# duanzhiihao/lossy-vae

Measured on AMD Instinct MI355X. Metric: Mpixels/s enc+dec (qarv_base, 512x768), higher is better.
Workload: dtype f32 (2-term fp16 split of every fp32 operand, hi + lo*2^-11 = 23 of 24 significant bits; 3 fp16 MFMAs per product step in two fp32 accumulators: fp32-class accuracy, parity-tested); 1 GPU; qarv_base batch=8 512x768 synthetic per GPU, compress_batch+decompress_batch, HIP kernels (f16x2) + host rANS, seeded random-init weights (profile typical); global_batch=8, parallelism=dp1 (images sharded, no data-path collective)

## Files before the change

lossy-vae_amd/csrc/gemm_h2_choice.h:

```cpp
#pragma once

#include "../../include/lvae_hip.h"

namespace lvae_h2 {

struct Choice {
    int kernel;
    int params[5];
    int splitk;
};

inline int slices(const lvae_gemm_desc& d) { return d.ksplit > 1 ? d.ksplit : 1; }

inline bool h2n_takes(const lvae_gemm_desc& d, bool force, Choice* c) {
    const bool conv3 = d.a_mode == LVAE_A_CONV3;
    if (d.prec != 4 || d.a_h2 || d.a_gelu || d.out_h2 || (d.a_mode != LVAE_A_PLAIN && !conv3) || d.N > 96 || (d.K & 15) || d.ldw != d.K) return false;
    if (!conv3 && (d.K1 != 0 || d.K0 != d.K || (d.lda0 & 3) || (long)d.M * d.lda0 * 4 > 0x7ffffff0L)) return false;
    if (conv3 && ((d.K0 & 15) || d.K != 9 * d.K0 || d.K1 != 0 || d.H <= 0 || d.W <= 0 || (long)d.M * d.K0 * 4 > 0x7ffffff0L)) return false;
    if ((long)d.N * d.K * 4 > 0x7ffffff0L) return false;
    const int S = slices(d);
    if (S > 1 && ((d.K / 16) % S || d.store != LVAE_ST_ROWMAJOR || (d.N & 3) || (d.ldo & 3) || (d.ldres & 3))) return false;
    if (!force && !(d.K & 16) && !(d.M >= 32768 && S == 1 && (conv3 || d.N > 64))) return false;
    *c = Choice{2, {(d.N + 31) / 32, conv3 ? LVAE_A_CONV3 : LVAE_A_PLAIN, 0, 0, 0}, 0};
    return true;
// ... 17 lines not shown
    if (sel <= 0 || sel > 2) {
        double best = 1e300;
        const double eff[3] = {0, 0.70, 1.00};
        for (int tn = 1; tn <= 2; ++tn) {
            const long tiles = (long)((M + 127) / 128) * ((N + 64 * tn - 1) / (64 * tn)) * S;
            const long rounds = (tiles + 511) / 512;
            const double cost = rounds * (128.0 * 64 * tn) * (K + 96.0) / eff[tn];
            if (cost < best) { best = cost; sel = tn; }
        }
    }
    *c = Choice{1, {sel, d.a_gelu ? 1 : 0, d.a_mode, 0, 0}, 0};
    return true;
}

inline bool h2p_takes(const lvae_gemm_desc& d, int force, int cu_count, Choice* c) {
    if (d.prec != 4 || !d.a_h2 || d.a_mode != LVAE_A_PLAIN || d.K1 != 0 || d.K0 != d.K || (d.K & 31) || d.lda0 != d.K ||
        d.ldw != d.K || d.a_gelu || (long)256 * d.K * 4 > 0x7fffffffL)
        return false;
    const int M = d.M, N = d.N;
    if (d.ksplit > 1) {
        if ((d.K / 32) % d.ksplit || d.store != LVAE_ST_ROWMAJOR || (N & 3) || (d.ldo & 3) || (d.ldres & 3)) return false;
        const int tiles = ((M + 127) / 128) * ((N + 63) / 64);
        const bool loaders = tiles <= cu_count;
        *c = Choice{3, {2, 1, 3, 1, loaders ? 8 : 0}, 0};
        return true;
    }
    int sel = force;
    if (sel != 42 && sel != 41 && sel != 22 && sel != 21 && sel != 23) {
        const int tn = (N % 128 == 0 || ((N + 127) / 128) * 128 - N < ((N + 63) / 64) * 64 - N + 1) ? 2 : 1;
        const long t128 = (long)((M + 127) / 128) * ((N + 127) / 128);
        sel = tn == 1 ? 21 : (t128 < 1024 ? 21 : (t128 >= 4096 ? 42 : 22));
        const long t64 = (long)((M + 127) / 128) * ((N + 63) / 64);
        if (d.K <= 512 && t64 >= 512 && (sel == 21 || (sel == 22 && t128 < 2048))) sel = 23;
    }
    switch (sel) {
        case 42: *c = Choice{3, {4, 2, 3, 0, 0}, 0}; break;
        case 41: *c = Choice{3, {4, 1, 3, 0, 0}, 0}; break;
        case 22: *c = Choice{3, {2, 2, 2, 0, 0}, 0}; break;
        case 23: *c = Choice{3, {2, 1, 2, 0, 0}, 0}; break;
        default: *c = Choice{3, {2, 1, 3, 0, 0}, 0}; break;
    }
    return true;
}

inline int family(const lvae_gemm_desc& d, int cu_count, Choice* c) {
    if (d.out_h2 && (d.store != LVAE_ST_ROWMAJOR || (d.epi != LVAE_EPI_BIAS && d.epi != LVAE_EPI_BIAS_GELU) || (d.N & 31) ||
                     d.ldo != d.N || (d.ksplit > 1 && !d.a_h2)))
        return -22;
    const int force = d.cfg > 0 ? d.cfg : 0;
    if (d.a_h2) return h2p_takes(d, force, cu_count, c) ? 0 : -22;
    return h2_takes(d, force, c) ? 0 : -22;
}

inline int choose(const lvae_gemm_desc& d, int cu_count, Choice* out) {
    if (d.prec != 4 || d.M <= 0 || d.N <= 0 || d.K <= 0 || (d.K & 7) || (d.ldw & 7)) return -22;
    if ((d.epi == LVAE_EPI_GAMMA_RES || d.epi == LVAE_EPI_RES) && !d.res) return -22;
    if (d.epi == LVAE_EPI_GAMMA_RES && !d.gamma) return -22;
    if (d.store != LVAE_ST_ROWMAJOR && (d.r <= 0 || d.N % (d.r * d.r) || d.H <= 0 || d.W <= 0)) return -22;
    const int S = slices(d);
    Choice c{};
    int rc;
    if (S == 1) {
        rc = family(d, cu_count, &c);
    } else if (d.a_h2) {
        if (d.store != LVAE_ST_ROWMAJOR || (d.N & 3) || (d.ldo & 3) || (d.ldres & 3) || d.K % (32 * S)) return -22;
        rc = family(d, cu_count, &c);
        c.splitk = 1;
    } else if ((d.cfg == 0 || d.cfg == 3) && h2n_takes(d, d.cfg == 3, &c)) {
        rc = 0;
        c.splitk = 1;
    } else {
        if (!d.ws || d.store != LVAE_ST_ROWMAJOR || (d.N & 3) || (d.ldo & 3) || (d.ldres & 3) || d.K % (32 * S)) return -22;
        rc = family(d, cu_count, &c);
        c.splitk = (d.cnt && ((d.N & 31) == 0 || d.N <= 32)) ? 2 : d.defer_reduce ? 4 : 3;
    }
    if (rc) return rc;
    *out = c;
    return 0;
// ... 4 lines not shown
```

lossy-vae_amd/csrc/gemm_h2p.hip:

```cpp
#include "gemm_common.h"

#include <type_traits>

namespace {

typedef _Float16 f16x8 __attribute__((ext_vector_type(8)));

#define LVAE_FENCE() __builtin_amdgcn_sched_barrier(0)
#define H2P_DSR(dst, addr, off) asm volatile("ds_read_b128 %0, %1 offset:%2" : "=v"(dst) : "v"(addr), "n"(off))
#define H2P_MFMA(a, b, c) __builtin_amdgcn_mfma_f32_32x32x16_f16(a, b, c, 0, 0, 0)

template <int WM, int TN, int NBUF, bool FOLD = false, int NLOAD = 0>
__global__ __launch_bounds__(128 * WM + 64 * NLOAD, (NLOAD ? 1 : (WM == 4 ? 1 : (NBUF == 2 && TN == 1 ? 3 : 2)))) void gemm_h2p_kernel(const lvae_gemm_desc d, int tiles_n, int n_tiles, int stagger) {
    using C = Cfg<WM, 2, 2, TN, 1, 32>;
    constexpr int BM = 64 * WM, BN = 64 * TN, ROWS = BM + BN, STAGE = ROWS * 128;
    constexpr int NWAVE = 2 * WM, NG = ROWS / 8, NI = NG / NWAVE;
    static_assert(NG % NWAVE == 0 && NWAVE % 2 == 0, "whole DMA instructions per wave; g has the parity of the wave");
    static_assert(NBUF * STAGE <= 160 * 1024 / (NLOAD ? 1 : (WM == 4 ? 1 : (NBUF == 2 && TN == 1 ? 3 : 2))), "LDS");
    static_assert(NLOAD == 0 || (NLOAD % 2 == 0 && NG % NLOAD == 0 && (NBUF - 2) * (NG / (NLOAD ? NLOAD : 1)) <= 63), "whole pieces per loader wave; the piece index has the loader's parity");
    extern __shared__ __attribute__((aligned(16))) float smem[];
    int t;
    {
        const int b = blockIdx.x, q = n_tiles / 8, r = n_tiles % 8, xcd = b % 8, loc = b / 8;
        t = (xcd < r ? xcd * (q + 1) : r * (q + 1) + (xcd - r) * q) + loc;
    }
    const int tm = t / tiles_n, tn = t - tm * tiles_n;
    const int m0 = tm * BM, n0 = tn * BN;
    const int tid = threadIdx.x, lane = tid & 63;
    const int wave = __builtin_amdgcn_readfirstlane(tid >> 6);
    const int wave_m = wave >> 1, wave_n = wave & 1;
    const int li = lane & 31, lh = lane >> 5;
    const int nq = d.K / 32;
    const int rowb = d.K * 4;
    if (stagger > 0) {
        const bool late = WM == 4 ? ((__builtin_amdgcn_s_getreg(((4 - 1) << 11) | (8 << 6) | 4) & 1) != 0)
                                  : (__builtin_amdgcn_s_getreg(((8 - 1) << 11) | (0 << 6) | 6) != 0);
        if (late)
            for (int i = 0; i < nq * stagger; ++i) __builtin_amdgcn_s_sleep(8);
    }

    const int rows_a = (d.M - m0) < BM ? (d.M - m0) : BM, rows_w = (d.N - n0) < BN ? (d.N - n0) : BN;
    const __amdgpu_buffer_rsrc_t rsA =
        __builtin_amdgcn_make_buffer_rsrc((void*)((const char*)d.A0 + (long)m0 * rowb), 0, rows_a * rowb, 0x00020000);
    const __amdgpu_buffer_rsrc_t rsW =
        __builtin_amdgcn_make_buffer_rsrc((void*)((const char*)d.Wt16 + (long)n0 * rowb), 0, rows_w * rowb, 0x00020000);
    if constexpr (NLOAD > 0) {
        if (wave >= NWAVE) {
// ... 12 lines not shown
                }
            };
#pragma unroll
            for (int s = 0; s < NBUF - 1; ++s) issue(s < nq ? s : nq - 1, s);
            int nb = NBUF - 1;
            for (int s = 0; s < nq; ++s) {
                asm volatile("s_waitcnt vmcnt(%0)\n\ts_barrier" ::"n"((NBUF - 2) * PL) : "memory");
                issue(s + NBUF - 1 < nq ? s + NBUF - 1 : nq - 1, nb);
                nb = nb == NBUF - 1 ? 0 : nb + 1;
            }
            asm volatile("s_waitcnt vmcnt(0)\n\ts_barrier" ::: "memory");
            return;
        }
    }
    const int r_in = lane >> 3, pp = lane & 7;
    const int dvoff = r_in * rowb + ((pp ^ ((4 * (wave & 1) + (r_in >> 1)) & 7)) << 4);
    auto dma = [&](int i, int stage, int buf) {
        const int g = i * NWAVE + wave;
        const bool isA = g < BM / 8;
        const int soff = (isA ? 8 * g : 8 * g - BM) * rowb + stage * 128;
        __builtin_amdgcn_raw_ptr_buffer_load_lds(isA ? rsA : rsW, (__attribute__((address_space(3))) void*)((char*)smem + buf * STAGE + g * 1024),
                                                 16, dvoff, soff, 0, 0);
    };

    const int xr = (li >> 1) & 7;
    unsigned a_base[4], b_base[4];
#pragma unroll
    for (int pt = 0; pt < 4; ++pt) {
        const int piece = 4 * (pt >> 1) + 2 * (pt & 1) + lh;
        const unsigned o = (unsigned)((piece ^ xr) << 4);
        a_base[pt] = (unsigned)(unsigned long)(__attribute__((address_space(3))) char*)((char*)smem) + (wave_m * 64 + li) * 128 + o;
        b_base[pt] = (unsigned)(unsigned long)(__attribute__((address_space(3))) char*)((char*)smem) + (BM + wave_n * 32 * TN + li) * 128 + o;
    }

    f32x16 accH[2][TN], accX[2][TN];
#pragma unroll
    for (int a = 0; a < 2; ++a)
// ... 12 lines not shown
            for (int a = 0; a < 2; ++a)
#pragma unroll
                for (int b = 0; b < TN; ++b)
#pragma unroll
                    for (int r = 0; r < 16; ++r) {
                        const float pr = __builtin_fmaf(accX[a][b][r], 1.0f / 2048.0f, accH[a][b][r]) + 0.0f;
                        tot[a][b][r] = slice == 0 ? pr : tot[a][b][r] + pr;
                        accH[a][b][r] = 0.f; accX[a][b][r] = 0.f;
                    }
            ++slice;
        }
    };

    if constexpr (NLOAD == 0) {
#pragma unroll
        for (int s = 0; s < NBUF - 1; ++s)
#pragma unroll
            for (int i = 0; i < NI; ++i) dma(i, s < nq ? s : nq - 1, s);
    }

    f16x8 af[2][2][2], bf[2][TN][2];
    auto stage_body = [&](auto buf_tag, int s) {
        constexpr int BUF = decltype(buf_tag)::value, NXT = (BUF + NBUF - 1) % NBUF;
        if constexpr (NLOAD > 0) asm volatile("s_barrier" ::: "memory");
        else asm volatile("s_waitcnt vmcnt(%0)\n\ts_barrier" ::"n"((NBUF - 2) * NI) : "memory");
        LVAE_FENCE();
        unsigned aa[4], ba[4];
#pragma unroll
        for (int pt = 0; pt < 4; ++pt) { aa[pt] = a_base[pt] + BUF * STAGE; ba[pt] = b_base[pt] + BUF * STAGE; }
#pragma unroll
        for (int tt = 0; tt < 2; ++tt) {
#pragma unroll
            for (int a = 0; a < 2; ++a) {
                H2P_DSR(af[tt][a][0], aa[0 + tt], a * 4096);
                H2P_DSR(af[tt][a][1], aa[2 + tt], a * 4096);
            }
#pragma unroll
            for (int b = 0; b < TN; ++b) {
                H2P_DSR(bf[tt][b][0], ba[0 + tt], b * 4096);
                H2P_DSR(bf[tt][b][1], ba[2 + tt], b * 4096);
            }
        }
        const int sn = s + NBUF - 1 < nq ? s + NBUF - 1 : nq - 1;
        int issued = 0;
#pragma unroll
        for (int tt = 0; tt < 2; ++tt) {
            if (tt == 0) {
                if constexpr (TN == 2) asm volatile("s_waitcnt lgkmcnt(8)" : "+v"(af[0][0][0]), "+v"(af[0][0][1]), "+v"(af[0][1][0]), "+v"(af[0][1][1]),
                                                    "+v"(bf[0][0][0]), "+v"(bf[0][0][1]), "+v"(bf[0][1][0]), "+v"(bf[0][1][1]));
                else asm volatile("s_waitcnt lgkmcnt(6)" : "+v"(af[0][0][0]), "+v"(af[0][0][1]), "+v"(af[0][1][0]), "+v"(af[0][1][1]),
                                  "+v"(bf[0][0][0]), "+v"(bf[0][0][1]));
            } else {
                if constexpr (TN == 2) asm volatile("s_waitcnt lgkmcnt(0)" : "+v"(af[1][0][0]), "+v"(af[1][0][1]), "+v"(af[1][1][0]), "+v"(af[1][1][1]),
                                                    "+v"(bf[1][0][0]), "+v"(bf[1][0][1]), "+v"(bf[1][1][0]), "+v"(bf[1][1][1]));
                else asm volatile("s_waitcnt lgkmcnt(0)" : "+v"(af[1][0][0]), "+v"(af[1][0][1]), "+v"(af[1][1][0]), "+v"(af[1][1][1]),
                                  "+v"(bf[1][0][0]), "+v"(bf[1][0][1]));
            }
            LVAE_FENCE();
// ... 6 lines not shown
                        accX[1][b] = H2P_MFMA(af[tt][1][1], bf[tt][b][0], accX[1][b]);
                    } else if (j == 1) {
                        accX[0][b] = H2P_MFMA(af[tt][0][0], bf[tt][b][1], accX[0][b]);
                        accX[1][b] = H2P_MFMA(af[tt][1][0], bf[tt][b][1], accX[1][b]);
                    } else {
                        accH[0][b] = H2P_MFMA(af[tt][0][0], bf[tt][b][0], accH[0][b]);
                        accH[1][b] = H2P_MFMA(af[tt][1][0], bf[tt][b][0], accH[1][b]);
                    }
                    if constexpr (NLOAD == 0) { if (issued < NI) { dma(issued, sn, NXT); ++issued; } }
                    LVAE_FENCE();
                }
            }
        }
        static_assert(NI <= 6 * TN, "DMA instructions per stage must fit the MFMA pairs of a stage");
    };
    for (int s = 0; s < nq; s += NBUF) {
        stage_body(std::integral_constant<int, 0>{}, s);
        fold();
        if (s + 1 < nq) { stage_body(std::integral_constant<int, 1 % NBUF>{}, s + 1); fold(); }
        if (NBUF > 2 && s + 2 < nq) { stage_body(std::integral_constant<int, 2 % NBUF>{}, s + 2); fold(); }
    }
    asm volatile("s_waitcnt vmcnt(0)\n\ts_barrier" ::: "memory");
    if constexpr (FOLD) {
        if (d.bias && n0 + BN <= d.N && !((d.ldo | d.ldres) & 3)) {
            if (d.epi == LVAE_EPI_BIAS_GELU && d.out_h2 && !(d.ldo & 31)) {
                h2p_epilogue_fast<TN, LVAE_EPI_BIAS_GELU, true, true, true>(d, tot, m0, n0, rows_a, wave_m, wave_n, li, lh);
                return;
            }
            if (d.epi == LVAE_EPI_GAMMA_RES && !d.out_h2) {
                h2p_epilogue_fast<TN, LVAE_EPI_GAMMA_RES, false, false, true>(d, tot, m0, n0, rows_a, wave_m, wave_n, li, lh);
                return;
            }
            if (d.epi == LVAE_EPI_RES && !d.out_h2) {
                h2p_epilogue_fast<TN, LVAE_EPI_RES, false, false, true>(d, tot, m0, n0, rows_a, wave_m, wave_n, li, lh);
                return;
            }
        }
        const int lj = li & 3;
#pragma unroll
        for (int a = 0; a < 2; ++a)
#pragma unroll
            for (int g = 0; g < 4; ++g) {
                const int row = m0 + (wave_m * 2 + a) * 32 + 4 * lh + 8 * g + lj;
// ... 1 lines not shown
                for (int b = 0; b < TN; ++b) {
                    float v0 = tot[a][b][4 * g + 0], v1 = tot[a][b][4 * g + 1], v2 = tot[a][b][4 * g + 2], v3 = tot[a][b][4 * g + 3];
                    quad_transpose(v0, v1, v2, v3, lj);
                    const int c4 = n0 + (wave_n * TN + b) * 32 + (li & ~3);
                    if (row < d.M && c4 < d.N) splitk_epilogue_store<true>(d, row, c4, (f32x4){v0, v1, v2, v3});
                }
            }
        return;
    }
#pragma unroll
    for (int a = 0; a < 2; ++a)
#pragma unroll
        for (int b = 0; b < TN; ++b)
#pragma unroll
            for (int r = 0; r < 16; ++r) accH[a][b][r] = __builtin_fmaf(accX[a][b][r], 1.0f / 2048.0f, accH[a][b][r]);
    if (d.store == LVAE_ST_ROWMAJOR && n0 + BN <= d.N && !((d.ldo | d.ldres) & 3)) {
        if (d.epi == LVAE_EPI_BIAS_GELU && d.out_h2 && !(d.ldo & 31)) {
            h2p_epilogue_fast<TN, LVAE_EPI_BIAS_GELU, true, true>(d, accH, m0, n0, rows_a, wave_m, wave_n, li, lh);
            return;
        }
        if (d.epi == LVAE_EPI_GAMMA_RES && !d.out_h2) {
            h2p_epilogue_fast<TN, LVAE_EPI_GAMMA_RES, false, false>(d, accH, m0, n0, rows_a, wave_m, wave_n, li, lh);
            return;
        }
        if (d.epi == LVAE_EPI_RES && !d.out_h2) {
            h2p_epilogue_fast<TN, LVAE_EPI_RES, false, false>(d, accH, m0, n0, rows_a, wave_m, wave_n, li, lh);
            return;
        }
    }
    gemm_finish<C>(d, accH, m0, n0, wave_m, wave_n, li, lh, (void*)smem, t);
}

template <int WM, int TN, int NBUF, bool FOLD = false, int NLOAD = 0>
int launch_h2p(const lvae_gemm_desc* d, hipStream_t st) {
    constexpr int BM = 64 * WM, BN = 64 * TN, LDS = NBUF * (BM + BN) * 128;
    static LdsAttr attr;
    if (const int ae = attr.ensure((const void*)gemm_h2p_kernel<WM, TN, NBUF, FOLD, NLOAD>, LDS)) return ae;
    const int tiles_m = (d->M + BM - 1) / BM, tiles_n = (d->N + BN - 1) / BN, n_tiles = tiles_m * tiles_n;
    hipLaunchKernelGGL((gemm_h2p_kernel<WM, TN, NBUF, FOLD, NLOAD>), dim3(n_tiles), dim3(128 * WM + 64 * NLOAD), LDS, st, *d, tiles_n, n_tiles, 0);
    return (int)hipGetLastError();
}

}

int lvae_gemm_h2p_launch(const lvae_gemm_desc* d, hipStream_t st, const int* params) {
    if (params[3]) return params[4] ? launch_h2p<2, 1, 3, true, 8>(d, st) : launch_h2p<2, 1, 3, true>(d, st);
    switch (100 * params[0] + 10 * params[1] + params[2]) {
        case 423: return launch_h2p<4, 2, 3>(d, st);
        case 413: return launch_h2p<4, 1, 3>(d, st);
        case 222: return launch_h2p<2, 2, 2>(d, st);
        case 212: return launch_h2p<2, 1, 2>(d, st);
        case 213: return launch_h2p<2, 1, 3>(d, st);
    }
    return -22;
}
```

lossy-vae_amd/lvae/engine.py:

```python
import ctypes

import torch

from . import _native
from ._native import GemmDesc


KSPLIT_MAX_TILES_PER_IMAGE = 96
KSPLIT_TARGET_WORKGROUPS = 256
INKERNEL_REDUCE_MAX_BYTES = 48 * 1024


def auto_ksplit(m1, N, K, store, ldo, ldres, prec):
    if store != _native.ST_ROWMAJOR or (N & 3) or (ldo & 3) or (ldres & 3) or K % 32:
        return 1
    nk = K // 32
    if prec == 1:
        if K % 64:
            return 1
        nk = K // 64
    tiles1 = ((m1 + 127) // 128) * ((N + 63) // 64)
    if tiles1 > KSPLIT_MAX_TILES_PER_IMAGE:
        return 1
    limit = min(nk // 4, KSPLIT_TARGET_WORKGROUPS // tiles1)
# ... 146 lines not shown
    def mlp_pipeline(self, C, hid, k, rows_per_image, n_affine=1):
        if self.mlp_h2p_ok(C, hid, k, n_affine, rows_per_image):
            return True, True, 1, 1
        if not self.mlp_h2p_ok(C, hid, k, n_affine, None):
            return False, False, None, None
        M = self.B * rows_per_image
        S1 = auto_ksplit(rows_per_image, hid, C, _native.ST_ROWMAJOR, hid, 0, 4)
        S2 = auto_ksplit(rows_per_image, C, hid, _native.ST_ROWMAJOR, C, C, 4)
        pre1 = self.serial_splitk_pays(M, hid, C, S1)
        pre2 = pre1 and self.serial_splitk_pays(M, C, hid, S2)
        return pre1, pre2, (S1 if pre1 else None), (S2 if pre2 else None)

    def mlp_q8_ok(self, C, hid, k, n_affine=1):
        return (self.prec == 3 and self.use_q8_pipeline and self.w16_q8 is not None and self.dwln_stores(3, C, k, n_affine)
                and C % 64 == 0 and hid % 64 == 0)

    def gemm(self, *, A0, K0, M, N, Wt, bias, out, lda0=None, A1=None, K1=0, lda1=0, ldw=None, ldo=None,
             gamma=None, res=None, ldres=0, a_mode=_native.A_PLAIN, epi=_native.EPI_BIAS, store=_native.ST_ROWMAJOR,
             r=0, H=0, W=0, K=None, a_gelu=0, Wt16=None, exact=False, ksplit=None, a_bf16=None, out_bf16=None, a_h2=False,
             out_h2=False, defer_reduce=False, label='gemm'):
        if K is None:
            K = K0 + K1
        if a_h2:
            assert self.prec in (3, 4) and Wt16 is None
            Wt16 = (self.w16_k32 if self.prec == 4 else self.w16_q8).get(Wt)
            assert Wt16, f'{label}: weights do not fit the pre-converted operand format'
        if Wt16 is None and self.w16 is not None:
            Wt16 = self.w16.get(Wt)
        d = GemmDesc()
        d.A0, d.A1 = A0, A1
        d.lda0, d.lda1 = (lda0 if lda0 is not None else K0), lda1
        d.K0, d.K1, d.H, d.W = K0, K1, H, W
        d.Wt, d.ldw = Wt, (ldw if ldw is not None else K)
        d.bias, d.gamma, d.res, d.ldres = bias, gamma, res, ldres
        d.out, d.ldo = out, (ldo if ldo is not None else N)
        d.M, d.N, d.K = M, N, K
        d.a_mode, d.epi, d.store, d.r = a_mode, epi, store, r
        d.status = self.status_ptr() if store == _native.ST_IMAGE else None
        d.cfg = 0
        d.a_gelu = a_gelu
        d.prec = (self.prec or 1) if (Wt16 and K % 8 == 0 and not exact) else 0
        d.a_h2, d.out_h2 = int(bool(a_h2)), int(bool(out_h2))
        if a_h2:
            assert a_mode == _native.A_PLAIN and K1 == 0 and K % (32 if self.prec == 4 else 64) == 0 and d.lda0 == K and d.ldw == K, label
            ksplit = (ksplit or 1) if self.prec == 4 else 1
            assert (K // 32) % ksplit == 0, label
        if out_h2:
            assert self.prec in (3, 4) and store == _native.ST_ROWMAJOR and N % (32 if self.prec == 4 else 64) == 0 and d.ldo == N, label
            if not a_h2:
                ksplit = 1
        if self.prec == 4 and not exact and not a_h2 and not (d.prec == 4 and self.lib.lvae_gemm_h2_choice(ctypes.byref(d), 256, None, None, None) == 0):
            Wt16 = self.w16_x3.get(Wt) if self.w16_x3 is not None else None
            d.prec = 2 if (Wt16 and K % 8 == 0) else 0
        d.Wt16 = Wt16 if d.prec else None
        if self.prec == 3:
            assert d.prec == 3, f'{label}: no MX-fp8 form of this GEMM (K={K})'
            d.ldw = K if a_h2 else (K + 63) // 64 * 64
            d.a_bf16 = 1 if a_bf16 is None else int(a_bf16)
            d.out_bf16 = (0 if store == _native.ST_IMAGE else 1) if out_bf16 is None else int(out_bf16)
            ksplit = 1
        if ksplit is None:
            ksplit = auto_ksplit(M // max(1, getattr(self, 'B', 1)), N, K, store, d.ldo, ldres, d.prec)
        deferred = None
        if ksplit > 1 and a_h2:
            d.ksplit = ksplit
        elif (1 < ksplit <= self.DEFER_MAX_PLANES and defer_reduce and epi == _native.EPI_BIAS and store == _native.ST_ROWMAJOR
              and d.ldo == N and bias):
            d.ksplit, d.ws, d.defer_reduce = ksplit, self.buf(self.sname('deferred_ws'), ksplit * M * N).data_ptr(), 1
            deferred = (d.ws, ksplit)
        elif ksplit > 1:
            d.ksplit, d.ws = ksplit, self.buf(self.sname('splitk_ws'), ksplit * M * N).data_ptr()
            if not deferred and ksplit * 128 * min(N, 192) * 4 <= INKERNEL_REDUCE_MAX_BYTES:
                n_cnt = ((M + 63) // 64) * ((N + 31) // 32)
                cname = self.sname('splitk_cnt')
                cnt = self.bufs.get(cname)
                if cnt is None or cnt.numel() < n_cnt:
                    if cnt is not None:
                        self.keep.append(cnt)
                    cnt = self.bufs[cname] = torch.zeros(max(4096, n_cnt), dtype=torch.int32, device=self.device)
                d.cnt = cnt.data_ptr()
        self.keep.append(d)
        self.flops += 2 * M * N * K
# ... 101 lines not shown
```

lossy-vae_amd/lvae/models/base.py:

```python
import ctypes
import functools
import logging
import math
import os
import threading
import time

import numpy as np
import torch
import torch.nn as nn

from .. import _native
from ..engine import NonFiniteError, Plan
from .entropy_coding import rans_decode_streams

_W16_LOCK = threading.Lock()


def split_bf16x3(t):
    hi = t.to(torch.bfloat16)
    r1 = t - hi.float()
    mid = r1.to(torch.bfloat16)
    lo = (r1 - mid.float()).to(torch.bfloat16)
    return torch.stack([hi, mid, lo], 0).contiguous()
# ... 155 lines not shown

    def alloc_symbols(self, n_sym, host=True):
        self.n_sym = n_sym
        self.sym_all, self.idx_all = self.new(n_sym, torch.int32), self.new(n_sym, torch.uint8)
        if host:
            self.sym_host = torch.empty(n_sym, dtype=torch.int32).pin_memory()
            self.idx_host = torch.empty(n_sym, dtype=torch.uint8).pin_memory()
            self.sym_np, self.idx_np = self.sym_host.numpy(), self.idx_host.numpy()

    def alloc_pos(self):
        self.pos_bufs = [self.new(self.B * hw, torch.float64) for _, hw in self.lat_shapes]

    def dwln_add(self, fmt, p, x, y, H, W, C, k):
        raise NotImplementedError

    def cnx(self, p, m, x, out, H, W):
        pk = self.pk
        C, k, hid = m.dim, m.kernel_size, m.hidden
        M = self.B * H * W
        y = self.buf(self.sname('y'), M * C, self.adt).data_ptr()
        mlp = dict(y=y, M=M, C=C, hid=hid, w1=pk.p(p + '.fc1_w'), b1=pk.p(p + '.fc1_b'), w2=pk.p(p + '.fc2_w'), b2=pk.p(p + '.fc2_b'),
                   gamma=pk.p(p + '.gamma'), res=x, out=out, label=p + '.mlp')
        if self.mlp_fused_ok(C, hid, k, M=M, rows_per_image=H * W):
            self.dwln_add('h2', p, x, y, H, W, C, k)
            self.mlp_fused(**mlp)
            return
        sk = self.mlp_sk_ok(C, hid, k, H * W, M) if self.use_mlp_sk else None
        if sk is not None:
            self.dwln_add('h2', p, x, y, H, W, C, k)
            self.mlp_sk(S1=sk[0], S2=sk[1], **mlp)
            return
        h = self.buf(self.sname('hid'), M * hid, self.adt).data_ptr()
        if self.mlp_q8_ok(C, hid, k):
            pre1, pre2, S1, S2 = True, True, None, None
        else:
            pre1, pre2, S1, S2 = self.mlp_pipeline(C, hid, k, H * W)
        fmt = ('q8' if pre1 else 'bf16') if self.lp else ('h2' if pre1 else 'f32')
        self.dwln_add(fmt, p, x, y, H, W, C, k)
        self.gemm(A0=y, K0=C, M=M, N=hid, Wt=pk.p(p + '.fc1_w'), bias=pk.p(p + '.fc1_b'), out=h,
                  epi=_native.EPI_BIAS_GELU, a_h2=pre1, out_h2=pre2, ksplit=S1, label=p + '.fc1')
        self.gemm(A0=h, K0=hid, M=M, N=C, Wt=pk.p(p + '.fc2_w'), bias=pk.p(p + '.fc2_b'),
                  gamma=pk.p(p + '.gamma'), res=x, ldres=C, out=out, epi=_native.EPI_GAMMA_RES, a_h2=pre2, ksplit=S2, label=p + '.fc2')


def on_model_device(fn):
    @functools.wraps(fn)
    def wrapper(self, *a, **k):
        dev = self._dummy.device
        if dev.type == 'cuda' and torch.cuda.current_device() != dev.index:
            with torch.cuda.device(dev):
                return fn(self, *a, **k)
        return fn(self, *a, **k)
    return wrapper


class CodecBase(nn.Module):
    def _init_codec_base(self):
# ... 840 lines not shown
```

lossy-vae_amd/lvae/models/qarv/model.py:

```python
import ctypes
import math
import os
import struct
import time
from collections import OrderedDict

import numpy as np
import torch
import torch.nn as nn

from ... import _native
from ...engine import ptr
from ...utils import coding
from ..base import CodecBase, CodecPlan, PackedWeights, on_model_device
from ..entropy_coding import DiscretizedGaussian, rans_encode_streams

EMBED_DIM = 256
SIDE_STREAM_MAX_PIXELS = 2 * 512 * 768


class _Marker(nn.Module):
    def __init__(self, kind, key=None):
        super().__init__()
        self.kind, self.key = kind, key
# ... 147 lines not shown

    def load_lmb(self, table, start):
        n = self.pk.adaln_total
        self.adaln_slab.copy_(table[start * n:(start + self.B) * n], non_blocking=True)

    def dwln_add(self, fmt, p, x, y, H, W, C, k):
        pk = self.pk
        off = pk.adaln_off[p]
        if self.vec:
            self.add(getattr(self.lib, f'lvae_dwconv_ln_{fmt}_v'), (x, pk.p(p + '.dw_w'), pk.p(p + '.dw_b'), ptr(self.adaln_slab, off),
                                                                   ptr(self.adaln_slab, off + C), y, self.B, H, W, C, k, pk.adaln_total), p + '.dwln')
        else:
            self.add(getattr(self.lib, f'lvae_dwconv_ln_{fmt}'), (x, pk.p(p + '.dw_w'), pk.p(p + '.dw_b'), None, None, ptr(pk.adaln, off),
                                                                 ptr(pk.adaln, off + C), y, self.B, H, W, C, k), p + '.dwln')

    def cnx(self, p, m, x, out, H, W):
        self.buf(self.sname('hid'), self.B * H * W * m.hidden, self.adt)
        super().cnx(p, m, x, out, H, W)

    def upsample(self, p, m, x, out, H, W, raw=False):
        pk = self.pk
        M = self.B * H * W
        final = m.cout <= 3
        if raw:
            assert final
            self.gemm(A0=x, K0=m.cin, M=M, N=m.cout * m.rate ** 2, Wt=pk.p(p + '.w_raw'), bias=pk.p(p + '.b_raw'), out=out,
                      store=_native.ST_SHUFFLE, r=m.rate, H=H, W=W, out_bf16=0, label=p + '.up_raw')
            return
        self.gemm(A0=x, K0=m.cin, M=M, N=m.cout * m.rate ** 2, Wt=pk.p(p + '.w'), bias=pk.p(p + '.b'), out=out,
                  store=_native.ST_IMAGE if final else _native.ST_SHUFFLE, r=m.rate, H=H, W=W, label=p + '.up')

    def prior(self, p, m, f, H, W, side_head=False):
        pk, lib, B = self.pk, self.lib, self.B
# ... 88 lines not shown
            elif m.kind == 'key':
                feats[m.key] = (x, h, w)
                tapped.add(x.data_ptr())
        h, w = H // 64, W // 64
        width = model.dec_blocks[0].width
        f = self.new(B * h * w * width, self.adt)
        self.add(lib.lvae_bias_expand_bf16 if self.lp else lib.lvae_bias_expand_f32, (pk.p('bias'), f.data_ptr(), B * h * w, width), 'bias')
        for i, m in enumerate(model.dec_blocks):
            p = f'dec_blocks.{i}'
            if m.kind == 'vrlv':
                M, z = B * h * w, m.zdim
                ef, eh, ew = feats[m.enc_key]
                assert (eh, ew) == (h, w)
                g = self.buf('post_g', M * m.width, self.adt)
                mg = self.buf('post_m', M * m.width, self.adt)
                if i in hoisted:
                    e = hoisted[i]
                else:
                    e = self.buf('post_e', M * m.enc_width, self.adt)
                    if small_side:
                        self.fork(p + '.fork_post0')
                        self.side_begin()
                    self.cnx(p + '.posterior0', m.posterior0, ef.data_ptr(), e.data_ptr(), h, w)
                    self.side_end()
                head_side = small_side
                pm, ioff = self.prior(p, m, f.data_ptr(), h, w, side_head=head_side)
                self.cnx(p + '.posterior1', m.posterior1, f.data_ptr(), g.data_ptr(), h, w)
                if head_side or i in hoisted:
                    self.join(p + '.join')
                self.gemm(A0=g.data_ptr(), K0=m.width, A1=e.data_ptr(), K1=m.enc_width, lda1=m.enc_width, M=M, N=m.width,
                          Wt=pk.p(p + '.post_merge.w'), bias=pk.p(p + '.post_merge.b'), out=mg.data_ptr(),
                          label=p + '.post_merge')
                self.cnx(p + '.posterior2', m.posterior2, mg.data_ptr(), mg.data_ptr(), h, w)
                qm = self.buf('qm', M * z)
                planes = self.gemm(A0=mg.data_ptr(), K0=m.width, M=M, N=z, K=9 * m.width, Wt=pk.p(p + '.posterior.w'),
                                   bias=pk.p(p + '.posterior.b'), out=qm.data_ptr(), a_mode=_native.A_CONV3, H=h, W=w, out_bf16=0,
                                   defer_reduce=(self.prec != 3 and self.DEFER_HEAD_REDUCE), label=p + '.posterior')
                zhat = self.buf('zhat', M * z)
                self.qm_bufs.append(qm); self.zhat_bufs.append(zhat); self.zhat_ld.append(z)
                self.sym_off.append(ioff)
                if planes:
                    self.add(lib.lvae_quantize_sk_f32, (planes[0], planes[1], pk.p(p + '.posterior.b'), qm.data_ptr(), pm.data_ptr(),
                                                        ptr(self.sym_all, ioff), zhat.data_ptr(), B, h * w, z, z, self.status_ptr()), p + '.quantize')
                else:
                    self.add(lib.lvae_quantize_f32, (qm.data_ptr(), pm.data_ptr(), ptr(self.sym_all, ioff), zhat.data_ptr(),
                                                     B, h * w, z, z, self.status_ptr()), p + '.quantize')
                self.qcuts.append(len(self.ops))
                if pos_bits:
                    self.lat_hw.append((h, w))
                if with_bits:
                    li = len(self.sym_off) - 1
                    self.add(lib.lvae_gaussian_nll_f32, (self.bufs['prm'].data_ptr(), ptr(self.sym_all, ioff), ptr(self.nats, li * B),
# ... 4 lines not shown
                    self.add(lib.lvae_gaussian_nll_chan_f32, (self.bufs['prm'].data_ptr(), ptr(self.sym_all, ioff), ptr(self.kl_chan, co),
                                                              pk.scale_bound, B, h * w, z, 0), p + '.nll_chan')
                self.fuse_and_end(p, m, f.data_ptr(), zhat.data_ptr(), h, w)
            elif m.kind == 'cnx':
                self.cnx(p, m, f.data_ptr(), f.data_ptr(), h, w)
            elif m.kind == 'up':
                nf = self.new(B * h * w * m.rate ** 2 * m.cout, self.adt)
                self.upsample(p, m, f.data_ptr(), nf.data_ptr(), h, w)
                f = nf
                h, w = h * m.rate, w * m.rate
            elif m.kind == 'stop':
                break
        if pos_bits:
            self.alloc_pos()

    def _hoist_posterior0(self, model, feats, hoisted, H, W):
        todo, s = [], 1
        for i, m in enumerate(model.dec_blocks):
            if m.kind == 'vrlv' and m.enc_key in feats:
                todo.append((i, m))
            elif m.kind == 'stop':
                break
        if not todo:
            return
        self.fork('hoist.fork')
        self.side_begin()
        for i, m in todo:
            ef, eh, ew = feats[m.enc_key]
            e = self.new(self.B * eh * ew * m.enc_width, self.adt)
            self.cnx(f'dec_blocks.{i}.posterior0', m.posterior0, ef.data_ptr(), e.data_ptr(), eh, ew)
            hoisted[i] = e
        self.side_end()


class _DecPlan(_NetPlan):

    def __init__(self, model, pk, B, nH, nW, evaluate=False, vec=False):
        super().__init__(model, pk, B, vec)
        lib = self.lib
        self.alloc_latent_io(nH, nW, host=not evaluate)
        h, w = nH, nW
        width = model.dec_blocks[0].width
        f = self.new(B * h * w * width, self.adt)
        self.add(lib.lvae_bias_expand_bf16 if self.lp else lib.lvae_bias_expand_f32, (pk.p('bias'), f.data_ptr(), B * h * w, width), 'bias')
        self.out = None
# ... 609 lines not shown
```

Measured before the change: 173.3 Mpixels/s.

## Emit pre-split fp16 activations into posterior merge and conv3 head GEMMs

Extends the pre-split (a_h2) GEMM kernel to take concatenated two-source A operands and gathered 3x3-conv A operands. The A tiles are loaded by DMA straight from per-tap offsets, with masking at image borders. The posterior ConvNeXt blocks' fc2 can now write the hi/lo fp16 split directly through a new GAMMA_RES out_h2 epilogue, so the post_merge GEMM (and optionally the head conv) skips re-splitting fp32 activations. The aim is to remove the conversion pass and reduce activation traffic. In exchange it adds kernel template variants and a per-tap buffer descriptor setup, and the head path stays off by default (HEAD_H2=False).

Result: no change. 172.9 Mpixels/s (-0.2%).

```diff
diff --git a/lossy-vae_amd/csrc/gemm_h2_choice.h b/lossy-vae_amd/csrc/gemm_h2_choice.h
--- a/lossy-vae_amd/csrc/gemm_h2_choice.h
+++ b/lossy-vae_amd/csrc/gemm_h2_choice.h
@@ -55,10 +55,24 @@
 }
 
 inline bool h2p_takes(const lvae_gemm_desc& d, int force, int cu_count, Choice* c) {
-    if (d.prec != 4 || !d.a_h2 || d.a_mode != LVAE_A_PLAIN || d.K1 != 0 || d.K0 != d.K || (d.K & 31) || d.lda0 != d.K ||
-        d.ldw != d.K || d.a_gelu || (long)256 * d.K * 4 > 0x7fffffffL)
+    const bool conv3 = d.a_mode == LVAE_A_CONV3, cat = d.a_mode == LVAE_A_PLAIN && d.K1 != 0;
+    if (d.prec != 4 || !d.a_h2 || (d.a_mode != LVAE_A_PLAIN && !conv3) || (d.K & 31) || d.ldw != d.K || d.a_gelu ||
+        (long)256 * d.K * 4 > 0x7fffffffL)
         return false;
+    if (conv3) {
+        if ((d.K0 & 31) || d.K0 <= 0 || d.K != 9 * d.K0 || d.K1 != 0 || d.H <= 0 || d.W <= 0 || (long)d.M * d.K0 * 4 > 0x7ffffff0L) return false;
+    } else if (cat) {
+        if (!d.A1 || (d.K0 & 31) || (d.K1 & 31) || d.K0 <= 0 || d.K1 < 0 || d.K0 + d.K1 != d.K || d.lda0 != d.K0 || d.lda1 != d.K1)
+            return false;
+    } else if (d.K0 != d.K || d.lda0 != d.K) {
+        return false;
+    }
     const int M = d.M, N = d.N;
+    if (conv3 || cat) {
+        if (d.ksplit > 1 && ((d.K / 32) % d.ksplit || d.store != LVAE_ST_ROWMAJOR || (N & 3) || (d.ldo & 3) || (d.ldres & 3))) return false;
+        *c = Choice{3, {2, 1, 3, d.ksplit > 1 ? 1 : 0, 0}, 0};
+        return true;
+    }
     if (d.ksplit > 1) {
         if ((d.K / 32) % d.ksplit || d.store != LVAE_ST_ROWMAJOR || (N & 3) || (d.ldo & 3) || (d.ldres & 3)) return false;
         const int tiles = ((M + 127) / 128) * ((N + 63) / 64);
@@ -85,8 +99,8 @@
 }
 
 inline int family(const lvae_gemm_desc& d, int cu_count, Choice* c) {
-    if (d.out_h2 && (d.store != LVAE_ST_ROWMAJOR || (d.epi != LVAE_EPI_BIAS && d.epi != LVAE_EPI_BIAS_GELU) || (d.N & 31) ||
-                     d.ldo != d.N || (d.ksplit > 1 && !d.a_h2)))
+    if (d.out_h2 && (d.store != LVAE_ST_ROWMAJOR || (d.epi != LVAE_EPI_BIAS && d.epi != LVAE_EPI_BIAS_GELU && d.epi != LVAE_EPI_GAMMA_RES) ||
+                     (d.epi == LVAE_EPI_GAMMA_RES && (d.ldres & 3)) || (d.N & 31) || d.ldo != d.N || (d.ksplit > 1 && !d.a_h2)))
         return -22;
     const int force = d.cfg > 0 ? d.cfg : 0;
     if (d.a_h2) return h2p_takes(d, force, cu_count, c) ? 0 : -22;
@@ -103,6 +117,11 @@
     int rc;
     if (S == 1) {
         rc = family(d, cu_count, &c);
+    } else if (d.a_h2 && d.a_mode == LVAE_A_CONV3 && d.defer_reduce && d.ws) {
+        if (d.store != LVAE_ST_ROWMAJOR || (d.N & 3) || (d.ldo & 3) || (d.ldres & 3) || d.K % (32 * S) || d.out_h2) return -22;
+        rc = family(d, cu_count, &c);
+        c.params[3] = 0;
+        c.splitk = 4;
     } else if (d.a_h2) {
         if (d.store != LVAE_ST_ROWMAJOR || (d.N & 3) || (d.ldo & 3) || (d.ldres & 3) || d.K % (32 * S)) return -22;
         rc = family(d, cu_count, &c);
diff --git a/lossy-vae_amd/csrc/gemm_h2p.hip b/lossy-vae_amd/csrc/gemm_h2p.hip
--- a/lossy-vae_amd/csrc/gemm_h2p.hip
+++ b/lossy-vae_amd/csrc/gemm_h2p.hip
@@ -10,7 +10,7 @@
 #define H2P_DSR(dst, addr, off) asm volatile("ds_read_b128 %0, %1 offset:%2" : "=v"(dst) : "v"(addr), "n"(off))
 #define H2P_MFMA(a, b, c) __builtin_amdgcn_mfma_f32_32x32x16_f16(a, b, c, 0, 0, 0)
 
-template <int WM, int TN, int NBUF, bool FOLD = false, int NLOAD = 0>
+template <int WM, int TN, int NBUF, bool FOLD = false, int NLOAD = 0, int AM = 0>
 __global__ __launch_bounds__(128 * WM + 64 * NLOAD, (NLOAD ? 1 : (WM == 4 ? 1 : (NBUF == 2 && TN == 1 ? 3 : 2)))) void gemm_h2p_kernel(const lvae_gemm_desc d, int tiles_n, int n_tiles, int stagger) {
     using C = Cfg<WM, 2, 2, TN, 1, 32>;
     constexpr int BM = 64 * WM, BN = 64 * TN, ROWS = BM + BN, STAGE = ROWS * 128;
@@ -18,6 +18,8 @@
     static_assert(NG % NWAVE == 0 && NWAVE % 2 == 0, "whole DMA instructions per wave; g has the parity of the wave");
     static_assert(NBUF * STAGE <= 160 * 1024 / (NLOAD ? 1 : (WM == 4 ? 1 : (NBUF == 2 && TN == 1 ? 3 : 2))), "LDS");
     static_assert(NLOAD == 0 || (NLOAD % 2 == 0 && NG % NLOAD == 0 && (NBUF - 2) * (NG / (NLOAD ? NLOAD : 1)) <= 63), "whole pieces per loader wave; the piece index has the loader's parity");
+    constexpr int NIA = BM / 8 / NWAVE;
+    static_assert(AM == 0 || (NLOAD == 0 && (BM / 8) % NWAVE == 0), "gathered A: the compute waves issue the DMA; A | W split at a whole instruction");
     extern __shared__ __attribute__((aligned(16))) float smem[];
     int t;
     {
@@ -31,6 +33,8 @@
     const int wave_m = wave >> 1, wave_n = wave & 1;
     const int li = lane & 31, lh = lane >> 5;
     const int nq = d.K / 32;
+    const int nst = AM ? nq / (int)gridDim.y : nq;
+    const int sbase = AM ? (int)blockIdx.y * nst : 0;
     const int rowb = d.K * 4;
     if (stagger > 0) {
         const bool late = WM == 4 ? ((__builtin_amdgcn_s_getreg(((4 - 1) << 11) | (8 << 6) | 4) & 1) != 0)
@@ -73,13 +77,62 @@
         }
     }
     const int r_in = lane >> 3, pp = lane & 7;
-    const int dvoff = r_in * rowb + ((pp ^ ((4 * (wave & 1) + (r_in >> 1)) & 7)) << 4);
+    const int pc = (pp ^ ((4 * (wave & 1) + (r_in >> 1)) & 7)) << 4;
+    const int dvoff = r_in * rowb + pc;
+    const int rowb0 = d.K0 * 4, rowb1 = d.K1 * 4, k0q = d.K0 / 32;
+    const int dvoff0 = r_in * rowb0 + pc, dvoff1 = r_in * rowb1 + pc;
+    int avoff[NIA], tapok[NIA];
+    int g_tap = 0, g_kk = 0, g_s = 0, g_toff = 0;
+    if constexpr (AM == 2) {
+#pragma unroll
+        for (int i = 0; i < NIA; ++i) {
+            const int m = m0 + 8 * (i * NWAVE + wave) + r_in;
+            const int w = m % d.W, h = (m / d.W) % d.H;
+            int ok = 0;
+#pragma unroll
+            for (int tp = 0; tp < 9; ++tp) {
+                const int hh = h + tp / 3 - 1, ww = w + tp % 3 - 1;
+                ok |= (m < d.M && hh >= 0 && hh < d.H && ww >= 0 && ww < d.W) ? (1 << tp) : 0;
+            }
+            tapok[i] = ok;
+            avoff[i] = m < d.M ? m * rowb0 + pc : 0;
+        }
+        g_tap = sbase / k0q;
+        g_kk = sbase - g_tap * k0q;
+    }
+    auto gather_at = [&](int stage) {
+        if constexpr (AM == 2) {
+            if (stage != g_s) {
+                ++g_s;
+                if (++g_kk == k0q) { g_kk = 0; ++g_tap; }
+            }
+            g_toff = ((g_tap / 3 - 1) * d.W + (g_tap % 3 - 1)) * rowb0 + g_kk * 128;
+            asm volatile("" : "+s"(g_toff));
+        }
+    };
     auto dma = [&](int i, int stage, int buf) {
         const int g = i * NWAVE + wave;
-        const bool isA = g < BM / 8;
-        const int soff = (isA ? 8 * g : 8 * g - BM) * rowb + stage * 128;
-        __builtin_amdgcn_raw_ptr_buffer_load_lds(isA ? rsA : rsW, (__attribute__((address_space(3))) void*)((char*)smem + buf * STAGE + g * 1024),
-                                                 16, dvoff, soff, 0, 0);
+        __attribute__((address_space(3))) void* dst = (__attribute__((address_space(3))) void*)((char*)smem + buf * STAGE + g * 1024);
+        if constexpr (AM == 0) {
+            const bool isA = g < BM / 8;
+            const int soff = (isA ? 8 * g : 8 * g - BM) * rowb + stage * 128;
+            __builtin_amdgcn_raw_ptr_buffer_load_lds(isA ? rsA : rsW, dst, 16, dvoff, soff, 0, 0);
+        } else {
+            const int sg = sbase + stage;
+            if (i >= NIA) {
+                __builtin_amdgcn_raw_ptr_buffer_load_lds(rsW, dst, 16, dvoff, (8 * g - BM) * rowb + sg * 128, 0, 0);
+            } else if constexpr (AM == 1) {
+                const bool second = sg >= k0q;
+                const int rb = second ? rowb1 : rowb0;
+                const __amdgpu_buffer_rsrc_t rs = __builtin_amdgcn_make_buffer_rsrc(
+                    (void*)((const char*)(second ? d.A1 : d.A0) + (long)m0 * rb), 0, rows_a * rb, 0x00020000);
+                __builtin_amdgcn_raw_ptr_buffer_load_lds(rs, dst, 16, second ? dvoff1 : dvoff0, 8 * g * rb + (second ? sg - k0q : sg) * 128, 0, 0);
+            } else {
+                const __amdgpu_buffer_rsrc_t rs = __builtin_amdgcn_make_buffer_rsrc((void*)d.A0, 0, d.M * rowb0, 0x00020000);
+                const int vo = ((tapok[i] >> g_tap) & 1) ? avoff[i] + g_toff : 0x7fffffff;
+                __builtin_amdgcn_raw_ptr_buffer_load_lds(rs, dst, 16, vo, 0, 0, 0);
+            }
+        }
     };
 
     const int xr = (li >> 1) & 7;
@@ -122,9 +175,11 @@
 
     if constexpr (NLOAD == 0) {
 #pragma unroll
-        for (int s = 0; s < NBUF - 1; ++s)
-#pragma unroll
-            for (int i = 0; i < NI; ++i) dma(i, s < nq ? s : nq - 1, s);
+        for (int s = 0; s < NBUF - 1; ++s) {
+            gather_at(s < nst ? s : nst - 1);
+#pragma unroll
+            for (int i = 0; i < NI; ++i) dma(i, s < nst ? s : nst - 1, s);
+        }
     }
 
     f16x8 af[2][2][2], bf[2][TN][2];
@@ -149,7 +204,8 @@
                 H2P_DSR(bf[tt][b][1], ba[2 + tt], b * 4096);
             }
         }
-        const int sn = s + NBUF - 1 < nq ? s + NBUF - 1 : nq - 1;
+        const int sn = s + NBUF - 1 < nst ? s + NBUF - 1 : nst - 1;
+        gather_at(sn);
         int issued = 0;
 #pragma unroll
         for (int tt = 0; tt < 2; ++tt) {
@@ -186,11 +242,11 @@
         }
         static_assert(NI <= 6 * TN, "DMA instructions per stage must fit the MFMA pairs of a stage");
     };
-    for (int s = 0; s < nq; s += NBUF) {
+    for (int s = 0; s < nst; s += NBUF) {
         stage_body(std::integral_constant<int, 0>{}, s);
         fold();
-        if (s + 1 < nq) { stage_body(std::integral_constant<int, 1 % NBUF>{}, s + 1); fold(); }
-        if (NBUF > 2 && s + 2 < nq) { stage_body(std::integral_constant<int, 2 % NBUF>{}, s + 2); fold(); }
+        if (s + 1 < nst) { stage_body(std::integral_constant<int, 1 % NBUF>{}, s + 1); fold(); }
+        if (NBUF > 2 && s + 2 < nst) { stage_body(std::integral_constant<int, 2 % NBUF>{}, s + 2); fold(); }
     }
     asm volatile("s_waitcnt vmcnt(0)\n\ts_barrier" ::: "memory");
     if constexpr (FOLD) {
@@ -199,6 +255,10 @@
                 h2p_epilogue_fast<TN, LVAE_EPI_BIAS_GELU, true, true, true>(d, tot, m0, n0, rows_a, wave_m, wave_n, li, lh);
                 return;
             }
+            if (d.epi == LVAE_EPI_GAMMA_RES && d.out_h2 && !(d.ldo & 31)) {
+                h2p_epilogue_fast<TN, LVAE_EPI_GAMMA_RES, true, true, true>(d, tot, m0, n0, rows_a, wave_m, wave_n, li, lh);
+                return;
+            }
             if (d.epi == LVAE_EPI_GAMMA_RES && !d.out_h2) {
                 h2p_epilogue_fast<TN, LVAE_EPI_GAMMA_RES, false, false, true>(d, tot, m0, n0, rows_a, wave_m, wave_n, li, lh);
                 return;
@@ -230,9 +290,13 @@
         for (int b = 0; b < TN; ++b)
 #pragma unroll
             for (int r = 0; r < 16; ++r) accH[a][b][r] = __builtin_fmaf(accX[a][b][r], 1.0f / 2048.0f, accH[a][b][r]);
-    if (d.store == LVAE_ST_ROWMAJOR && n0 + BN <= d.N && !((d.ldo | d.ldres) & 3)) {
+    if ((AM == 0 || gridDim.y == 1) && d.store == LVAE_ST_ROWMAJOR && n0 + BN <= d.N && !((d.ldo | d.ldres) & 3)) {
         if (d.epi == LVAE_EPI_BIAS_GELU && d.out_h2 && !(d.ldo & 31)) {
             h2p_epilogue_fast<TN, LVAE_EPI_BIAS_GELU, true, true>(d, accH, m0, n0, rows_a, wave_m, wave_n, li, lh);
+            return;
+        }
+        if (d.epi == LVAE_EPI_GAMMA_RES && d.out_h2 && !(d.ldo & 31)) {
+            h2p_epilogue_fast<TN, LVAE_EPI_GAMMA_RES, true, true>(d, accH, m0, n0, rows_a, wave_m, wave_n, li, lh);
             return;
         }
         if (d.epi == LVAE_EPI_GAMMA_RES && !d.out_h2) {
@@ -257,9 +321,24 @@
     return (int)hipGetLastError();
 }
 
+template <int AM, bool FOLD>
+int launch_gathered(const lvae_gemm_desc* d, hipStream_t st, int slices) {
+    constexpr int LDS = 3 * (128 + 64) * 128;
+    static LdsAttr attr;
+    if (const int ae = attr.ensure((const void*)gemm_h2p_kernel<2, 1, 3, FOLD, 0, AM>, LDS)) return ae;
+    const int tiles_n = (d->N + 63) / 64, n_tiles = ((d->M + 127) / 128) * tiles_n;
+    hipLaunchKernelGGL((gemm_h2p_kernel<2, 1, 3, FOLD, 0, AM>), dim3(n_tiles, slices), dim3(256), LDS, st, *d, tiles_n, n_tiles, 0);
+    return (int)hipGetLastError();
+}
+
 }
 
 int lvae_gemm_h2p_launch(const lvae_gemm_desc* d, hipStream_t st, const int* params) {
+    if (d->a_mode == LVAE_A_CONV3 || d->K1 != 0) {
+        if (params[0] != 2 || params[1] != 1 || params[2] != 3 || params[4]) return -22;
+        if (d->a_mode != LVAE_A_CONV3) return params[3] ? launch_gathered<1, true>(d, st, 1) : launch_gathered<1, false>(d, st, 1);
+        return params[3] ? launch_gathered<2, true>(d, st, 1) : launch_gathered<2, false>(d, st, d->ksplit > 1 ? d->ksplit : 1);
+    }
     if (params[3]) return params[4] ? launch_h2p<2, 1, 3, true, 8>(d, st) : launch_h2p<2, 1, 3, true>(d, st);
     switch (100 * params[0] + 10 * params[1] + params[2]) {
         case 423: return launch_h2p<4, 2, 3>(d, st);
diff --git a/lossy-vae_amd/lvae/engine.py b/lossy-vae_amd/lvae/engine.py
--- a/lossy-vae_amd/lvae/engine.py
+++ b/lossy-vae_amd/lvae/engine.py
@@ -184,6 +184,25 @@
     def mlp_q8_ok(self, C, hid, k, n_affine=1):
         return (self.prec == 3 and self.use_q8_pipeline and self.w16_q8 is not None and self.dwln_stores(3, C, k, n_affine)
                 and C % 64 == 0 and hid % 64 == 0)
+
+    def a_h2_ok(self, *, M, N, K0, Wt, K1=0, a_mode=_native.A_PLAIN, H=0, W=0, defer_reduce=False):
+        K = 9 * K0 if a_mode == _native.A_CONV3 else K0 + K1
+        if self.prec != 4 or self.w16_k32 is None or K % 32 or not self.w16.get(Wt) or not self.w16_k32.get(Wt):
+            return False
+        S = auto_ksplit(M // max(1, getattr(self, 'B', 1)), N, K, _native.ST_ROWMAJOR, N, 0, 4)
+        if S > 1 and K1 and not self.serial_splitk_pays(M, N, K, S):
+            return False
+        for a_h2 in (0, 1):
+            d = GemmDesc()
+            d.M, d.N, d.K, d.K0, d.K1, d.H, d.W, d.a_mode, d.prec = M, N, K, K0, K1, H, W, a_mode, 4
+            d.lda0, d.lda1, d.ldw, d.ldo, d.a_h2 = K0, K1, K, N, a_h2
+            d.A1 = 1 if K1 else None
+            if S > 1:
+                d.ksplit, d.ws = S, 1
+                d.defer_reduce = int(bool(defer_reduce) and S <= self.DEFER_MAX_PLANES)
+            if self.lib.lvae_gemm_h2_choice(ctypes.byref(d), 256, None, None, None) != 0:
+                return False
+        return True
 
     def gemm(self, *, A0, K0, M, N, Wt, bias, out, lda0=None, A1=None, K1=0, lda1=0, ldw=None, ldo=None,
              gamma=None, res=None, ldres=0, a_mode=_native.A_PLAIN, epi=_native.EPI_BIAS, store=_native.ST_ROWMAJOR,
@@ -211,7 +230,10 @@
         d.a_gelu = a_gelu
         d.prec = (self.prec or 1) if (Wt16 and K % 8 == 0 and not exact) else 0
         d.a_h2, d.out_h2 = int(bool(a_h2)), int(bool(out_h2))
-        if a_h2:
+        gathered = bool(a_h2) and self.prec == 4 and (a_mode == _native.A_CONV3 or K1 != 0)
+        if gathered:
+            assert K0 % 32 == 0 and K1 % 32 == 0 and d.ldw == K and (a_mode == _native.A_CONV3 or (d.lda0 == K0 and lda1 == K1)), label
+        elif a_h2:
             assert a_mode == _native.A_PLAIN and K1 == 0 and K % (32 if self.prec == 4 else 64) == 0 and d.lda0 == K and d.ldw == K, label
             ksplit = (ksplit or 1) if self.prec == 4 else 1
             assert (K // 32) % ksplit == 0, label
@@ -232,10 +254,11 @@
         if ksplit is None:
             ksplit = auto_ksplit(M // max(1, getattr(self, 'B', 1)), N, K, store, d.ldo, ldres, d.prec)
         deferred = None
-        if ksplit > 1 and a_h2:
+        defer_ok = (1 < ksplit <= self.DEFER_MAX_PLANES and defer_reduce and epi == _native.EPI_BIAS and store == _native.ST_ROWMAJOR
+                    and d.ldo == N and bias)
+        if ksplit > 1 and a_h2 and not (gathered and defer_ok):
             d.ksplit = ksplit
-        elif (1 < ksplit <= self.DEFER_MAX_PLANES and defer_reduce and epi == _native.EPI_BIAS and store == _native.ST_ROWMAJOR
-              and d.ldo == N and bias):
+        elif defer_ok:
             d.ksplit, d.ws, d.defer_reduce = ksplit, self.buf(self.sname('deferred_ws'), ksplit * M * N).data_ptr(), 1
             deferred = (d.ws, ksplit)
         elif ksplit > 1:
diff --git a/lossy-vae_amd/lvae/models/base.py b/lossy-vae_amd/lvae/models/base.py
--- a/lossy-vae_amd/lvae/models/base.py
+++ b/lossy-vae_amd/lvae/models/base.py
@@ -193,7 +193,17 @@
     def dwln_add(self, fmt, p, x, y, H, W, C, k):
         raise NotImplementedError
 
-    def cnx(self, p, m, x, out, H, W):
+    def cnx_out_h2_ok(self, m, H, W):
+        C, k, hid = m.dim, m.kernel_size, m.hidden
+        M = self.B * H * W
+        if self.prec != 4 or C % 32 or self.mlp_fused_ok(C, hid, k, M=M, rows_per_image=H * W):
+            return False
+        if self.use_mlp_sk and self.mlp_sk_ok(C, hid, k, H * W, M) is not None:
+            return False
+        return bool(self.mlp_pipeline(C, hid, k, H * W)[1])
+
+    def cnx(self, p, m, x, out, H, W, out_h2=False):
+        assert not out_h2 or (self.cnx_out_h2_ok(m, H, W) and out != x), p
         pk = self.pk
         C, k, hid = m.dim, m.kernel_size, m.hidden
         M = self.B * H * W
@@ -219,7 +229,8 @@
         self.gemm(A0=y, K0=C, M=M, N=hid, Wt=pk.p(p + '.fc1_w'), bias=pk.p(p + '.fc1_b'), out=h,
                   epi=_native.EPI_BIAS_GELU, a_h2=pre1, out_h2=pre2, ksplit=S1, label=p + '.fc1')
         self.gemm(A0=h, K0=hid, M=M, N=C, Wt=pk.p(p + '.fc2_w'), bias=pk.p(p + '.fc2_b'),
-                  gamma=pk.p(p + '.gamma'), res=x, ldres=C, out=out, epi=_native.EPI_GAMMA_RES, a_h2=pre2, ksplit=S2, label=p + '.fc2')
+                  gamma=pk.p(p + '.gamma'), res=x, ldres=C, out=out, epi=_native.EPI_GAMMA_RES, a_h2=pre2, out_h2=out_h2, ksplit=S2,
+                  label=p + '.fc2')
 
 
 def on_model_device(fn):
diff --git a/lossy-vae_amd/lvae/models/qarv/model.py b/lossy-vae_amd/lvae/models/qarv/model.py
--- a/lossy-vae_amd/lvae/models/qarv/model.py
+++ b/lossy-vae_amd/lvae/models/qarv/model.py
@@ -185,9 +185,9 @@
             self.add(getattr(self.lib, f'lvae_dwconv_ln_{fmt}'), (x, pk.p(p + '.dw_w'), pk.p(p + '.dw_b'), None, None, ptr(pk.adaln, off),
                                                                  ptr(pk.adaln, off + C), y, self.B, H, W, C, k), p + '.dwln')
 
-    def cnx(self, p, m, x, out, H, W):
+    def cnx(self, p, m, x, out, H, W, **kw):
         self.buf(self.sname('hid'), self.B * H * W * m.hidden, self.adt)
-        super().cnx(p, m, x, out, H, W)
+        super().cnx(p, m, x, out, H, W, **kw)
 
     def upsample(self, p, m, x, out, H, W, raw=False):
         pk = self.pk
@@ -306,6 +306,7 @@
                 assert (eh, ew) == (h, w)
                 g = self.buf('post_g', M * m.width, self.adt)
                 mg = self.buf('post_m', M * m.width, self.adt)
+                merge_h2, head_h2 = self.merge_h2(p, m, h, w), self.head_h2(p, m, h, w)
                 if i in hoisted:
                     e = hoisted[i]
                 else:
@@ -313,21 +314,22 @@
                     if small_side:
                         self.fork(p + '.fork_post0')
                         self.side_begin()
-                    self.cnx(p + '.posterior0', m.posterior0, ef.data_ptr(), e.data_ptr(), h, w)
+                    self.cnx(p + '.posterior0', m.posterior0, ef.data_ptr(), e.data_ptr(), h, w, out_h2=merge_h2)
                     self.side_end()
                 head_side = small_side
                 pm, ioff = self.prior(p, m, f.data_ptr(), h, w, side_head=head_side)
-                self.cnx(p + '.posterior1', m.posterior1, f.data_ptr(), g.data_ptr(), h, w)
+                self.cnx(p + '.posterior1', m.posterior1, f.data_ptr(), g.data_ptr(), h, w, out_h2=merge_h2)
                 if head_side or i in hoisted:
                     self.join(p + '.join')
                 self.gemm(A0=g.data_ptr(), K0=m.width, A1=e.data_ptr(), K1=m.enc_width, lda1=m.enc_width, M=M, N=m.width,
-                          Wt=pk.p(p + '.post_merge.w'), bias=pk.p(p + '.post_merge.b'), out=mg.data_ptr(),
+                          Wt=pk.p(p + '.post_merge.w'), bias=pk.p(p + '.post_merge.b'), out=mg.data_ptr(), a_h2=merge_h2,
                           label=p + '.post_merge')
-                self.cnx(p + '.posterior2', m.posterior2, mg.data_ptr(), mg.data_ptr(), h, w)
+                mh = self.buf('post_mh', M * m.width, self.adt) if head_h2 else mg
+                self.cnx(p + '.posterior2', m.posterior2, mg.data_ptr(), mh.data_ptr(), h, w, out_h2=head_h2)
                 qm = self.buf('qm', M * z)
-                planes = self.gemm(A0=mg.data_ptr(), K0=m.width, M=M, N=z, K=9 * m.width, Wt=pk.p(p + '.posterior.w'),
+                planes = self.gemm(A0=mh.data_ptr(), K0=m.width, M=M, N=z, K=9 * m.width, Wt=pk.p(p + '.posterior.w'),
                                    bias=pk.p(p + '.posterior.b'), out=qm.data_ptr(), a_mode=_native.A_CONV3, H=h, W=w, out_bf16=0,
-                                   defer_reduce=(self.prec != 3 and self.DEFER_HEAD_REDUCE), label=p + '.posterior')
+                                   defer_reduce=(self.prec != 3 and self.DEFER_HEAD_REDUCE), a_h2=head_h2, label=p + '.posterior')
                 zhat = self.buf('zhat', M * z)
                 self.qm_bufs.append(qm); self.zhat_bufs.append(zhat); self.zhat_ld.append(z)
                 self.sym_off.append(ioff)
@@ -362,6 +364,17 @@
         if pos_bits:
             self.alloc_pos()
 
+    MERGE_H2, HEAD_H2 = True, False
+
+    def merge_h2(self, p, m, h, w):
+        return (self.MERGE_H2 and self.prec == 4 and self.cnx_out_h2_ok(m.posterior1, h, w) and self.cnx_out_h2_ok(m.posterior0, h, w)
+                and self.a_h2_ok(M=self.B * h * w, N=m.width, K0=m.width, K1=m.enc_width, Wt=self.pk.p(p + '.post_merge.w')))
+
+    def head_h2(self, p, m, h, w):
+        return (self.HEAD_H2 and self.prec == 4 and self.cnx_out_h2_ok(m.posterior2, h, w)
+                and self.a_h2_ok(M=self.B * h * w, N=m.zdim, K0=m.width, a_mode=_native.A_CONV3, H=h, W=w,
+                                 Wt=self.pk.p(p + '.posterior.w'), defer_reduce=self.DEFER_HEAD_REDUCE))
+
     def _hoist_posterior0(self, model, feats, hoisted, H, W):
         todo, s = [], 1
         for i, m in enumerate(model.dec_blocks):
@@ -376,7 +389,7 @@
         for i, m in todo:
             ef, eh, ew = feats[m.enc_key]
             e = self.new(self.B * eh * ew * m.enc_width, self.adt)
-            self.cnx(f'dec_blocks.{i}.posterior0', m.posterior0, ef.data_ptr(), e.data_ptr(), eh, ew)
+            self.cnx(f'dec_blocks.{i}.posterior0', m.posterior0, ef.data_ptr(), e.data_ptr(), eh, ew, out_h2=self.merge_h2(f'dec_blocks.{i}', m, eh, ew))
             hoisted[i] = e
         self.side_end()
 
```
